# nexus1203/libBICOS

Measured on NVIDIA B200. Metric: Mpx/s disparity, higher is better.
Workload: dtype u8

## Files before the change

libbicos_b200/csrc/search_mma.cu:

```cuda

#include "kernels.cuh"

#include <atomic>
#include <limits.h>
#include <mutex>
#include <stdio.h>
#include <stdlib.h>
#include <string.h>

namespace bicos_b200 {
namespace {

constexpr int TM = 128;
constexpr int TN = 128;
constexpr int NTHREADS = 320;
constexpr int ATOM_BYTES = 128 * 128;
constexpr uint32_t TMEM_COLS = 2 * TN;
constexpr int COL_BITS = 13;
constexpr int COL_MAX = (1 << COL_BITS) - 1;
#ifndef BICOS_MMA_COLTERM_DEFAULT
#define BICOS_MMA_COLTERM_DEFAULT 1
#endif

__device__ __forceinline__ uint32_t smem_u32(const void* p) {
// ... 132 lines not shown
    asm volatile(
        "tcgen05.ld.sync.aligned.32x32b.x32.b32 {%0, %1, %2, %3, %4, %5, %6, %7, %8, %9, %10, %11, %12, %13, %14, %15, %16, %17, %18, %19, %20, %21, %22, %23, %24, %25, %26, %27, %28, %29, %30, %31}, [%32];"
        : "=r"(v[0]), "=r"(v[1]), "=r"(v[2]), "=r"(v[3]), "=r"(v[4]), "=r"(v[5]), "=r"(v[6]), "=r"(v[7]), "=r"(v[8]), "=r"(v[9]), "=r"(v[10]), "=r"(v[11]), "=r"(v[12]), "=r"(v[13]), "=r"(v[14]), "=r"(v[15]), "=r"(v[16]), "=r"(v[17]), "=r"(v[18]), "=r"(v[19]), "=r"(v[20]), "=r"(v[21]), "=r"(v[22]), "=r"(v[23]), "=r"(v[24]), "=r"(v[25]), "=r"(v[26]), "=r"(v[27]), "=r"(v[28]), "=r"(v[29]), "=r"(v[30]), "=r"(v[31])
        : "r"(taddr)
        : "memory"
    );
}

__device__ __forceinline__ void tc_load64_packed_issue(uint32_t taddr, int (&v)[32]) {
    asm volatile(
        "tcgen05.ld.sync.aligned.32x32b.x32.pack::16b.b32 {%0, %1, %2, %3, %4, %5, %6, %7, %8, %9, %10, %11, %12, %13, %14, %15, %16, %17, %18, %19, %20, %21, %22, %23, %24, %25, %26, %27, %28, %29, %30, %31}, [%32];"
        : "=r"(v[0]), "=r"(v[1]), "=r"(v[2]), "=r"(v[3]), "=r"(v[4]), "=r"(v[5]), "=r"(v[6]), "=r"(v[7]), "=r"(v[8]), "=r"(v[9]), "=r"(v[10]), "=r"(v[11]), "=r"(v[12]), "=r"(v[13]), "=r"(v[14]), "=r"(v[15]), "=r"(v[16]), "=r"(v[17]), "=r"(v[18]), "=r"(v[19]), "=r"(v[20]), "=r"(v[21]), "=r"(v[22]), "=r"(v[23]), "=r"(v[24]), "=r"(v[25]), "=r"(v[26]), "=r"(v[27]), "=r"(v[28]), "=r"(v[29]), "=r"(v[30]), "=r"(v[31])
        : "r"(taddr)
        : "memory"
    );
}

__device__ __forceinline__ void tc_load32_wait(int (&v)[32]) {
    asm volatile("tcgen05.wait::ld.sync.aligned;" : "+r"(v[0]), "+r"(v[1]), "+r"(v[2]), "+r"(v[3]), "+r"(v[4]), "+r"(v[5]), "+r"(v[6]), "+r"(v[7]), "+r"(v[8]), "+r"(v[9]), "+r"(v[10]), "+r"(v[11]), "+r"(v[12]), "+r"(v[13]), "+r"(v[14]), "+r"(v[15]), "+r"(v[16]), "+r"(v[17]), "+r"(v[18]), "+r"(v[19]), "+r"(v[20]), "+r"(v[21]), "+r"(v[22]), "+r"(v[23]), "+r"(v[24]), "+r"(v[25]), "+r"(v[26]), "+r"(v[27]), "+r"(v[28]), "+r"(v[29]), "+r"(v[30]), "+r"(v[31])::"memory");
}

__device__ __forceinline__ void tc_store32(uint32_t taddr, const uint32_t (&v)[32]) {
    asm volatile(
        "tcgen05.st.sync.aligned.32x32b.x32.b32 [%0], {%1, %2, %3, %4, %5, %6, %7, %8, %9, %10, %11, %12, %13, %14, %15, %16, %17, %18, %19, %20, %21, %22, %23, %24, %25, %26, %27, %28, %29, %30, %31, %32};"
        :
        : "r"(taddr), "r"(v[0]), "r"(v[1]), "r"(v[2]), "r"(v[3]), "r"(v[4]), "r"(v[5]), "r"(v[6]), "r"(v[7]), "r"(v[8]), "r"(v[9]), "r"(v[10]), "r"(v[11]), "r"(v[12]), "r"(v[13]), "r"(v[14]), "r"(v[15]), "r"(v[16]), "r"(v[17]), "r"(v[18]), "r"(v[19]), "r"(v[20]), "r"(v[21]), "r"(v[22]), "r"(v[23]), "r"(v[24]), "r"(v[25]), "r"(v[26]), "r"(v[27]), "r"(v[28]), "r"(v[29]), "r"(v[30]), "r"(v[31])
        : "memory"
    );
}

__device__ __forceinline__ void tc_store_wait() {
    asm volatile("tcgen05.wait::st.sync.aligned;" ::: "memory");
}

__device__ __forceinline__ void tc_mma_i8_ts(uint32_t tmem_d, uint32_t tmem_a, uint64_t bdesc, uint32_t idesc, uint32_t accumulate) {
    asm volatile(
        "{\n"
        ".reg .pred p;\n"
        "setp.ne.b32 p, %4, 0;\n"
        "tcgen05.mma.cta_group::1.kind::i8 [%0], [%1], %2, %3, p;\n"
        "}"
        :
        : "r"(tmem_d), "r"(tmem_a), "l"(bdesc), "r"(idesc), "r"(accumulate)
        : "memory"
    );
}

__device__ __forceinline__ uint64_t smem_desc(uint32_t saddr) {
    uint64_t d = (uint64_t)((saddr & 0x3FFFFu) >> 4);
    d |= (uint64_t)1 << 16;
    d |= (uint64_t)(1024 >> 4) << 32;
    d |= (uint64_t)1 << 46;
    d |= (uint64_t)2 << 61;
    return d;
}

constexpr uint32_t IDESC = (2u << 4) | (1u << 7) | (0u << 10) | ((uint32_t)(TN >> 3) << 17) | ((uint32_t)(TM >> 4) << 24);

__device__ __forceinline__ void st_shared_v4(uint32_t addr, uint32_t a, uint32_t b, uint32_t c, uint32_t d) {
    asm volatile("st.shared.v4.b32 [%0], {%1, %2, %3, %4};" ::"r"(addr), "r"(a), "r"(b), "r"(c), "r"(d) : "memory");
}

template<bool RIGHT, int S>
__device__ __forceinline__ uint32_t expand_word(uint32_t w) {
    if constexpr (RIGHT) {
        if constexpr (S == 0)
            return (w << 7) & 0x80808080u;
        else
            return w & (0x01010101u << S);
    } else {
        constexpr int P = S == 0 ? 0 : 7 - S;
        constexpr uint32_t MAG = 0x01010101u << P;
        constexpr uint32_t HIGH = 0x01010101u * ((0xFFu << (P + 1)) & 0xFFu);
        const uint32_t neg = ((w >> S) & 0x01010101u) * 0xFFu;
        return (neg & HIGH) | MAG;
    }
}

template<int K, bool RIGHT, bool CT = false>
__device__ __forceinline__ void expand_pixel(const uint4 (&d)[K / 4], uint32_t tile, int r) {
    const uint32_t row = tile + (uint32_t)r * 128u;
    const uint32_t sw = (uint32_t)(r & 7);
#pragma unroll
    for (int q = 0; q < K / 4; ++q) {
        const uint32_t w[4] = { d[q].x, d[q].y, d[q].z, d[q].w };
#pragma unroll
        for (int wi = 0; wi < 4; ++wi) {
            st_shared_v4(
                row + (uint32_t)q * ATOM_BYTES + ((((uint32_t)(2 * wi)) ^ sw) << 4),
                expand_word<RIGHT, 0>(w[wi]),
                expand_word<RIGHT, 1>(w[wi]),
                expand_word<RIGHT, 2>(w[wi]),
                expand_word<RIGHT, 3>(w[wi])
            );
            st_shared_v4(
                row + (uint32_t)q * ATOM_BYTES + ((((uint32_t)(2 * wi + 1)) ^ sw) << 4),
                expand_word<RIGHT, 4>(w[wi]),
                expand_word<RIGHT, 5>(w[wi]),
                expand_word<RIGHT, 6>(w[wi]),
                (RIGHT && CT && q == K / 4 - 1 && wi == 3) ? (expand_word<RIGHT, 7>(w[wi]) | ((uint32_t)r << 24)) : expand_word<RIGHT, 7>(w[wi])
            );
        }
    }
}

template<int K>
// ... 666 lines not shown
                    TileMin16 m;
                    tc_load64_packed_issue(acc, va);
                    tc_load64_packed_issue(acc + 64, vb);
                    tc_load32_wait(va);
                    tc_load32_wait(vb);
                    tc_fence_before();
                    mbar_arrive(bar_acc_drained + 8 * (2 * a + h));
                    fold64_packed<NODUPES, 0, CT>(va, m);
                    fold64_packed<NODUPES, 64, CT>(vb, m);
                    merge_tile<NODUPES>(m, tile0, m_first, m_last);
                } else {
                    TileMin32 m;
                    tc_load32_issue(acc, va);
                    tc_load32_wait(va);
                    tc_load32_issue(acc + 32, vb);
                    fold32<NODUPES, 0, CT>(va, m);
                    tc_load32_wait(vb);
                    tc_load32_issue(acc + 64, va);
                    fold32<NODUPES, 32, CT>(vb, m);
                    tc_load32_wait(va);
                    tc_load32_issue(acc + 96, vb);
                    fold32<NODUPES, 64, CT>(va, m);
                    tc_load32_wait(vb);
                    tc_fence_before();
                    mbar_arrive(bar_acc_drained + 8 * (2 * a + h));
                    fold32<NODUPES, 96, CT>(vb, m);
                    merge_tile<NODUPES>(m, tile0, m_first, m_last);
                }
                if (n + 1 < nitems && t == (NA == 2 ? min(2, ntiles - 1) : ntiles - 1))
                    pa_next = stage_left(dl, n + 1);
            }
            const int i = it.mt * 2 * TM + h * TM + lane128;
            if (i < cols) {
                const size_t at = (size_t)it.row * cols + i;
                (it.dir ? p.rev_first : p.fwd_first)[at] = ((uint32_t)(pa + (m_first >> COL_BITS)) << 16) | ((uint32_t)m_first & COL_MAX);
                if constexpr (NODUPES)
                    (it.dir ? p.rev_last : p.fwd_last)[at] =
                        ((uint32_t)(pa + (m_last >> COL_BITS)) << 16) | ((65535u - COL_MAX) + ((uint32_t)m_last & COL_MAX));
            }
            it = nx;
        }
    }

teardown:
    tc_fence_before();
    __syncthreads();
    if (warp == 1) {
        tc_fence_after();
        asm volatile("tcgen05.dealloc.cta_group::1.sync.aligned.b32 %0, %1;" ::"r"(*(volatile uint32_t*)&tmem_base_slot), "r"(512u) : "memory");
    }
}

constexpr int V3_THREADS = 512;
template<int K>
constexpr int V3_REGS_LAUNCH = K == 4 ? 104 : 112;
constexpr int V3_REGS_EPILOGUE = 168;
template<int K>
constexpr int V3_REGS_PRODUCER = K == 4 ? 40 : 56;
template<int K>
constexpr int V3_REGS_ISSUER = K == 4 ? 40 : 56;
template<int K>
constexpr bool V3_REGS_FIT = 256 * V3_REGS_EPILOGUE + 128 * V3_REGS_PRODUCER<K> + 128 * V3_REGS_ISSUER<K> <= V3_THREADS * V3_REGS_LAUNCH<K>;
static_assert(V3_REGS_FIT<4> && V3_REGS_FIT<8>, "register budget");
template<int K>
constexpr int V3_ASLOTS = K == 4 ? 4 : 2;
constexpr int V3_PACKED = 4;
constexpr uint32_t V3_A_COL0 = 3 * TN;
template<int K>
constexpr int V3_PACKED_BYTES = TN * K * 4;
template<int K>
constexpr int V3_OFFSET = K == 4 ? 0 : 16384;
constexpr int V3_STATE_STRIDE = 132;
constexpr int V3_STATE_BYTES = 64 * V3_STATE_STRIDE * 4;
constexpr int V3_FIN_BYTES = 2 * TN * 4;
template<int K>
constexpr int V3_SMEM_BYTES = 4 * (K / 4) * ATOM_BYTES + V3_PACKED * V3_PACKED_BYTES<K> + 2 * V3_STATE_BYTES + 2 * V3_FIN_BYTES + 1024;
static_assert(V3_SMEM_BYTES<8> <= 227 * 1024, "shared memory");
constexpr uint32_t IDESC3 = (2u << 4) | (0u << 7) | (1u << 10) | ((uint32_t)(TN >> 3) << 17) | ((uint32_t)(TM >> 4) << 24);

__device__ __forceinline__ void tc_store8(uint32_t taddr, const uint32_t (&v)[8]) {
    asm volatile("tcgen05.st.sync.aligned.32x32b.x8.b32 [%0], {%1, %2, %3, %4, %5, %6, %7, %8};" ::"r"(taddr), "r"(v[0]), "r"(v[1]), "r"(v[2]),
                 "r"(v[3]), "r"(v[4]), "r"(v[5]), "r"(v[6]), "r"(v[7])
                 : "memory");
}

__device__ __forceinline__ void st_shared_v2(uint32_t addr, uint32_t a, uint32_t b) {
    asm volatile("st.shared.v2.b32 [%0], {%1, %2};" ::"r"(addr), "r"(a), "r"(b) : "memory");
}
__device__ __forceinline__ void st_shared_u32(uint32_t addr, uint32_t a) {
    asm volatile("st.shared.b32 [%0], %1;" ::"r"(addr), "r"(a) : "memory");
}
__device__ __forceinline__ uint32_t ld_shared_u32(uint32_t addr) {
    uint32_t v;
    asm volatile("ld.shared.b32 %0, [%1];" : "=r"(v) : "r"(addr) : "memory");
    return v;
}
__device__ __forceinline__ uint32_t pinned(uint32_t v) {
    uint32_t r;
    asm volatile("mov.u32 %0, %1;" : "=r"(r) : "r"(v));
    return r;
}

template<int K>
__device__ __forceinline__ void expand_moving_to_tmem(const uint4 (&d)[K / 4], uint32_t taddr) {
#pragma unroll
    for (int q = 0; q < K / 4; ++q) {
    const uint32_t w[4] = { d[q].x, d[q].y, d[q].z, d[q].w };
#pragma unroll
    for (int wi = 0; wi < 4; ++wi) {
        uint32_t v[8];
        v[0] = expand_word<true, 0>(w[wi]);
        v[1] = expand_word<true, 1>(w[wi]);
        v[2] = expand_word<true, 2>(w[wi]);
        v[3] = expand_word<true, 3>(w[wi]);
        v[4] = expand_word<true, 4>(w[wi]);
        v[5] = expand_word<true, 5>(w[wi]);
        v[6] = expand_word<true, 6>(w[wi]);
        v[7] = expand_word<true, 7>(w[wi]);
        if (q == K / 4 - 1 && wi == 3) {
            v[6] |= 128u << 24;
            v[7] |= 1u << 24;
        }
        tc_store8(taddr + 32u * q + 8u * wi, v);
    }
    }
    tc_store_wait();
}

template<int K>
__device__ __forceinline__ void expand_block_pixel(const uint4 (&d)[K / 4], uint32_t tile, int r) {
    const uint32_t row = tile + (uint32_t)r * 128u;
    const uint32_t sw = (uint32_t)(r & 7);
    int pc = 0;
#pragma unroll
    for (int q = 0; q < K / 4; ++q)
        pc += __popc(d[q].x) + __popc(d[q].y) + __popc(d[q].z) + __popc(d[q].w);
    const uint32_t pc_byte = (uint32_t)(pc - (K == 4 ? 0 : 128)) & 0xFFu;
#pragma unroll
    for (int q = 0; q < K / 4; ++q) {
        const uint32_t w[4] = { d[q].x, d[q].y, d[q].z, d[q].w };
        const uint32_t atom = row + (uint32_t)q * ATOM_BYTES;
#pragma unroll
        for (int wi = 0; wi < 4; ++wi) {
            st_shared_v4(atom + ((((uint32_t)(2 * wi)) ^ sw) << 4), expand_word<false, 0>(w[wi]), expand_word<false, 1>(w[wi]),
                         expand_word<false, 2>(w[wi]), expand_word<false, 3>(w[wi]));
            uint32_t s6 = expand_word<false, 6>(w[wi]), s7 = expand_word<false, 7>(w[wi]);
            if (q == K / 4 - 1 && wi == 3) {
                s6 = (s6 & 0x00FFFFFFu) | (pc_byte << 24);
                s7 = (s7 & 0x00FFFFFFu) | ((uint32_t)r << 24);
            }
            st_shared_v4(atom + ((((uint32_t)(2 * wi + 1)) ^ sw) << 4), expand_word<false, 4>(w[wi]), expand_word<false, 5>(w[wi]), s6, s7);
        }
    }
}

template<int L>
__device__ __forceinline__ uint32_t key_of_hi(uint32_t w, uint32_t mask) {
    uint32_t k;
    asm("lop3.b32 %0, %1, %2, %3, 0xEA;" : "=r"(k) : "r"(w), "r"(mask), "n"(L));
    return k;
}
template<int L4>
struct ReduceLanes {
    static __device__ __forceinline__ void run(uint32_t src, uint32_t mask, uint32_t shl16, uint32_t& mlo, uint32_t& mhi) {
        const uint4 w = ld_shared_v4(src + 16u * L4);
        mhi = min(mhi, min(key_of_hi<4 * L4>(w.x, mask), key_of_hi<4 * L4 + 1>(w.y, mask)));
        mlo = min(mlo, min(w.x * shl16 + (uint32_t)(4 * L4), w.y * shl16 + (uint32_t)(4 * L4 + 1)));
        mhi = min(mhi, min(key_of_hi<4 * L4 + 2>(w.z, mask), key_of_hi<4 * L4 + 3>(w.w, mask)));
        mlo = min(mlo, min(w.z * shl16 + (uint32_t)(4 * L4 + 2), w.w * shl16 + (uint32_t)(4 * L4 + 3)));
        ReduceLanes<L4 + 1>::run(src, mask, shl16, mlo, mhi);
    }
};
template<>
struct ReduceLanes<16> {
    static __device__ __forceinline__ void run(uint32_t, uint32_t, uint32_t, uint32_t&, uint32_t&) {}
};

#define V3_ROLE_CONTEXT \
    uint32_t fresh; \
    asm volatile("mov.u32 %0, 0;" : "=r"(fresh)); \
    const uint32_t tmem = *(volatile uint32_t*)&tmem_base_slot + fresh; \
    const int cols = p.cols; \
    const int ntiles = p.ntiles;  \
    const int npairs = p.mtiles;  \
    const long long item0 = p.items * (blockIdx.x + fresh) / gridDim.x; \
    const int nitems = (int)(p.items * (blockIdx.x + fresh + 1) / gridDim.x - item0); \
    const uint32_t s_blk = ((smem_u32(smem_raw) + fresh) + 1023u) & ~1023u;  \
    const uint32_t s_packed = s_blk + 4 * BLK_BYTES; \
    const uint32_t s_state = s_packed + NP * PACKED_BYTES;  \
    const uint32_t s_fin = s_state + 2 * V3_STATE_BYTES;  \
    const uint32_t bar_packed_full = smem_u32(&bars[0]) + fresh; \
    const uint32_t bar_packed_free = bar_packed_full + 8 * NP; \
    const uint32_t bar_a_full = bar_packed_free + 8 * NP; \
    const uint32_t bar_a_free = bar_a_full + 8 * NS; \
    const uint32_t bar_blk_full = bar_a_free + 8 * NS;  \
    const uint32_t bar_blk_free = bar_blk_full + 32; \
    const uint32_t bar_acc_full = bar_blk_free + 32; \
    const uint32_t bar_acc_drained = bar_acc_full + 48; \
    const uint32_t bar_epi = bar_acc_drained + 48;  \
    int row = (int)(item0 / npairs), bp = (int)(item0 - (long long)row * npairs); \
    (void)tmem, (void)cols, (void)ntiles, (void)s_blk, (void)s_packed, (void)s_state, (void)s_fin, (void)bar_packed_full, (void)bar_packed_free, \
        (void)bar_a_full, (void)bar_a_free, (void)bar_blk_full, (void)bar_blk_free, (void)bar_acc_full, (void)bar_acc_drained, (void)bar_epi, \
        (void)row, (void)bp;

template<int K>
__global__ void __maxnreg__(V3_REGS_LAUNCH<K>) search_mma3_kernel(const MmaArgs p) {
    constexpr int KA = K / 4;
    constexpr int NS = V3_ASLOTS<K>;
    constexpr int NP = V3_PACKED;
    constexpr int PACKED_BYTES = V3_PACKED_BYTES<K>;
    constexpr int BLK_BYTES = KA * ATOM_BYTES;
    constexpr uint32_t A_COLS = 32u * KA;
    constexpr int OFF = V3_OFFSET<K>;
    extern __shared__ uint8_t smem_raw[];
    __shared__ uint64_t bars[2 * NP + 2 * NS + 8 + 12 + 2];
    __shared__ uint32_t tmem_base_slot;
    __shared__ Watch s_watch;

    const int tid = threadIdx.x;
    const int warp = tid >> 5;

    if (tid == 0) {
        const uint32_t bar0 = smem_u32(&bars[0]);
        s_watch.flag = p.timeout_flag;
        s_watch.timeout_ns = p.timeout_ns;
        s_watch.abort = 0;
        for (int s = 0; s < NP; ++s) {
            mbar_init(bar0 + 8 * s, 1);
            mbar_init(bar0 + 8 * (NP + s), TM);
        }
        for (int s = 0; s < NS; ++s) {
            mbar_init(bar0 + 8 * (2 * NP + s), TM);
            mbar_init(bar0 + 8 * (2 * NP + NS + s), 2);
        }
        for (int b = 0; b < 4; ++b) {
            mbar_init(bar0 + 8 * (2 * NP + 2 * NS + b), TN);
            mbar_init(bar0 + 8 * (2 * NP + 2 * NS + 4 + b), 1);
        }
        for (int a = 0; a < 6; ++a) {
            mbar_init(bar0 + 8 * (2 * NP + 2 * NS + 8 + a), 1);
            mbar_init(bar0 + 8 * (2 * NP + 2 * NS + 14 + a), TM);
        }
        mbar_init(bar0 + 8 * (2 * NP + 2 * NS + 20), TM);
        mbar_init(bar0 + 8 * (2 * NP + 2 * NS + 21), TM);
        asm volatile("fence.mbarrier_init.release.cluster;" ::: "memory");
    }
    if (warp == 1) {
        asm volatile("tcgen05.alloc.cta_group::1.sync.aligned.shared::cta.b32 [%0], %1;" ::"r"(smem_u32(&tmem_base_slot)), "r"(512u)
                     : "memory");
        asm volatile("tcgen05.relinquish_alloc_permit.cta_group::1.sync.aligned;" ::: "memory");
    }
    tc_fence_before();
    __syncthreads();
    tc_fence_after();

    if (warp >= 12) {
        regs_shrink<V3_REGS_ISSUER<K>>();
        V3_ROLE_CONTEXT
    if (warp == 15) {
    } else if (warp == 12 || warp == 13) {
        {
            const int h = warp - 12;
            const uint32_t u_tmem = uniform(tmem);
            const uint64_t desc_b0 = smem_desc(uniform(s_blk)) + (uint32_t)h * (uint32_t)(BLK_BYTES >> 4);
            constexpr uint32_t BUFFER_STEP = (2 * BLK_BYTES) >> 4;
            uint32_t s = 0, a_phase = 0;
            uint32_t a = (uint32_t)h, d6 = (uint32_t)h + 3u, d_phase = 1u;
            int q = h;
            for (int n = 0; n < nitems; ++n) {
                const uint32_t b = (uint32_t)n & 1u;
                if (!mbar_wait(bar_blk_full + 8 * (2 * b + h), ((uint32_t)n >> 1) & 1u, &s_watch))
                    goto teardown;
                const uint64_t desc_b = desc_b0 + b * BUFFER_STEP;
                for (int t = 0; t < ntiles; ++t, q += 2) {
                    if (!mbar_wait(bar_a_full + 8 * s, a_phase, &s_watch))
                        goto teardown;
                    if (q >= 3)
                        if (!mbar_wait(bar_acc_drained + 8 * (2 * a + (1 - h)), d_phase, &s_watch))
                            goto teardown;
                    tc_fence_after();
                    if (elect_one()) {
#pragma unroll
                        for (int qa = 0; qa < KA; ++qa)
#pragma unroll
                            for (int kk = 0; kk < 4; ++kk)
                                tc_mma_i8_ts(u_tmem + a * TN, u_tmem + V3_A_COL0 + s * A_COLS + (uint32_t)(qa * 32 + kk * 8),
                                             desc_b + (uint32_t)((qa * ATOM_BYTES + kk * 32) >> 4), IDESC3, (qa | kk) != 0);
                        tc_commit(bar_acc_full + 8 * (2 * a + h));
                        tc_commit(bar_a_free + 8 * s);
                    }
                    __syncwarp();
                    if (++s == NS) {
                        s = 0;
                        a_phase ^= 1u;
                    }
                    a = a == 0 ? 2u : a - 1u;
                    d6 += 2u;
                    if (d6 >= 6u) {
                        d6 -= 6u;
                        d_phase ^= 1u;
                    }
                }
                if (elect_one())
                    tc_commit(bar_blk_free + 8 * (2 * b + h));
                __syncwarp();
            }
        }
    } else if (warp == 14) {
        if (tid == 14 * 32) {
            uint32_t slot = 0, free_phase = 1u;
            bool wrapped = false;
            const uint32_t tail_bytes = (uint32_t)(cols - (ntiles - 1) * TN) * (uint32_t)(K * 4);
            auto put = [&](const uint32_t* src, uint32_t bytes) -> bool {
                if (wrapped)
                    if (!mbar_wait(bar_packed_free + 8 * slot, free_phase, &s_watch))
                        return false;
                mbar_expect_tx(bar_packed_full + 8 * slot, bytes);
                bulk_copy_g2s(s_packed + slot * (uint32_t)PACKED_BYTES, src, bytes, bar_packed_full + 8 * slot);
                if (++slot == (uint32_t)NP) {
                    slot = 0;
                    free_phase ^= 1u;
                    wrapped = true;
                }
                return true;
            };
            for (int n = 0; n < nitems; ++n) {
                const uint32_t* const lrow = p.left + (size_t)row * p.pitch_words;
                const uint32_t* const rrow = p.right + (size_t)row * p.pitch_words;
                for (int e = 0; e < 2; ++e) {
                    const int base = min((2 * bp + e) * TN, cols - 1);
                    if (!put(rrow + (size_t)base * K, (uint32_t)min(TN, cols - base) * (uint32_t)(K * 4)))
                        goto teardown;
                }
                for (int t = 0; t < ntiles - 1; ++t)
                    if (!put(lrow + (size_t)t * (TN * K), (uint32_t)PACKED_BYTES))
                        goto teardown;
                if (!put(lrow + (size_t)(ntiles - 1) * (TN * K), tail_bytes))
                    goto teardown;
                if (++bp == npairs) {
                    bp = 0;
                    ++row;
                }
            }
        }
    }
    } else if (warp >= 8) {
        regs_shrink<V3_REGS_PRODUCER<K>>();
        V3_ROLE_CONTEXT
        const int r = (int)pinned((uint32_t)(tid - 2 * TM));
        const uint32_t lane_base = tmem + ((uint32_t)((warp & 3) * 32) << 16);
        uint32_t ps = 0, full_phase = 0, as = 0, a_free_phase = 1u;
        bool a_wrapped = false;
        const uint32_t my_px = s_packed + (uint32_t)r * (uint32_t)(K * 4);
        const uint32_t my_tail_px = s_packed + (uint32_t)min(r, cols - (ntiles - 1) * TN - 1) * (uint32_t)(K * 4);
        for (int n = 0; n < nitems; ++n) {
            for (int e = 0; e < 2; ++e) {
                const int valid = min(TN, cols - min((2 * bp + e) * TN, cols - 1));
                if (!mbar_wait(bar_packed_full + 8 * ps, full_phase, &s_watch))
                    goto teardown;
                uint4 d[KA];
                {
                    const uint32_t src = s_packed + ps * (uint32_t)PACKED_BYTES + (uint32_t)min(r, valid - 1) * (uint32_t)(K * 4);
#pragma unroll
                    for (int q = 0; q < KA; ++q)
                        d[q] = ld_shared_v4(src + 16u * q);
                }
                const uint32_t b = 2u * ((uint32_t)n & 1u) + (uint32_t)e;
                if (n >= 2)
                    if (!mbar_wait(bar_blk_free + 8 * b, (((uint32_t)n >> 1) - 1u) & 1u, &s_watch))
                        goto teardown;
                expand_block_pixel<K>(d, s_blk + b * BLK_BYTES, r);
                mbar_arrive(bar_packed_free + 8 * ps);
                fence_async_smem();
                mbar_arrive(bar_blk_full + 8 * b);
                if (++ps == (uint32_t)NP) {
                    ps = 0;
                    full_phase ^= 1u;
                }
            }
            for (int t = 0; t < ntiles; ++t) {
                if (!mbar_wait(bar_packed_full + 8 * ps, full_phase, &s_watch))
                    goto teardown;
                uint4 d[KA];
                {
                    const uint32_t src = (t == ntiles - 1 ? my_tail_px : my_px) + ps * (uint32_t)PACKED_BYTES;
#pragma unroll
                    for (int q = 0; q < KA; ++q)
                        d[q] = ld_shared_v4(src + 16u * q);
                }
                if (a_wrapped)
                    if (!mbar_wait(bar_a_free + 8 * as, a_free_phase, &s_watch))
                        goto teardown;
                tc_fence_after();
                expand_moving_to_tmem<K>(d, lane_base + V3_A_COL0 + as * A_COLS);
                mbar_arrive(bar_packed_free + 8 * ps);
                tc_fence_before();
                mbar_arrive(bar_a_full + 8 * as);
                if (++ps == (uint32_t)NP) {
                    ps = 0;
                    full_phase ^= 1u;
                }
                if (++as == (uint32_t)NS) {
                    as = 0;
                    a_free_phase ^= 1u;
                    a_wrapped = true;
                }
            }
            if (++bp == npairs) {
                bp = 0;
                ++row;
            }
        }
    } else {
        regs_grow<V3_REGS_EPILOGUE>();
        V3_ROLE_CONTEXT
        const int h = (int)pinned((uint32_t)(warp >> 2));
        const int lane128 = (int)pinned((uint32_t)(tid & (TM - 1)));
        const uint32_t lane_base = tmem + ((uint32_t)((warp & 3) * 32) << 16);
        const uint32_t my_state = s_state + (uint32_t)(h * V3_STATE_BYTES);
        const uint32_t my_fin = s_fin + (uint32_t)(h * V3_FIN_BYTES);
        const uint32_t my_epi = bar_epi + 8u * (uint32_t)h;
        uint32_t R[64];
#pragma unroll
        for (int c = 0; c < 64; ++c)
            R[c] = 0x7FFF7FFFu;
        uint32_t epi_phase = 0;
        uint32_t a = (uint32_t)h, acc_phase = 0;
        int lo[32], hi[32];
        int left = nitems * ntiles;
        if (left > 0) {
            if (!mbar_wait(bar_acc_full + 8 * (2 * a + h), acc_phase, &s_watch))
                goto teardown;
            tc_fence_after();
            tc_load64_packed_issue(lane_base + a * TN, lo);
            --left;
        }
        for (int n = 0; n < nitems; ++n) {
            const size_t row_at = (size_t)row * cols;
            const int col0 = (2 * bp + h) * TN;
            const int fwd_cols = col0 < cols ? cols : 0;
            for (int t = 0; t < ntiles; ++t) {
                const uint32_t tile2 = (uint32_t)(t + OFF) * 0x00010001u;
                uint32_t f[8];
                tc_load32_wait(lo);
                tc_load64_packed_issue(lane_base + a * TN + 64u, hi);
#pragma unroll
                for (int c = 0; c < 8; ++c)
                    f[c] = __vimin3_s16x2((uint32_t)lo[c], (uint32_t)lo[8 + c], (uint32_t)lo[16 + c]);
#pragma unroll
                for (int c = 0; c < 4; ++c)
                    f[c] = __vimin3_s16x2(f[c], (uint32_t)lo[24 + 2 * c], (uint32_t)lo[25 + 2 * c]);
#pragma unroll
                for (int c = 0; c < 32; ++c)
                    R[c] = __viaddmin_s16x2((uint32_t)lo[c], tile2, R[c]);
                tc_load32_wait(hi);
                tc_fence_before();
                mbar_arrive(bar_acc_drained + 8 * (2 * a + h));
                a = a == 0 ? 2u : a - 1u;
                if (a == (uint32_t)h)
                    acc_phase ^= 1u;
                if (left > 0) {
                    if (!mbar_wait(bar_acc_full + 8 * (2 * a + h), acc_phase, &s_watch))
                        goto teardown;
                    tc_fence_after();
                    tc_load64_packed_issue(lane_base + a * TN, lo);
                    --left;
                }
#pragma unroll
                for (int c = 0; c < 8; ++c)
                    f[c] = __vimin3_s16x2(f[c], (uint32_t)hi[c], (uint32_t)hi[8 + c]);
#pragma unroll
                for (int c = 0; c < 8; ++c)
                    f[c] = __vimin3_s16x2(f[c], (uint32_t)hi[16 + c], (uint32_t)hi[24 + c]);
                const uint32_t m2 = __vimin3_s16x2(__vimin3_s16x2(f[0], f[1], f[2]), __vimin3_s16x2(f[3], f[4], f[5]), __vmins2(f[6], f[7]));
                const uint32_t m = OFF ? (uint32_t)(min((int)(short)(m2 & 0xFFFFu), (int)(short)(m2 >> 16)) + OFF) : min(m2 & 0xFFFFu, m2 >> 16);
                const int i = t * TM + lane128;
                if (i < fwd_cols)
                    atomicMin(p.fwd_first + row_at + i, m * 512u + (uint32_t)col0 - (m & 127u) * 511u);
#pragma unroll
                for (int c = 0; c < 32; ++c)
                    R[32 + c] = __viaddmin_s16x2((uint32_t)hi[c], tile2, R[32 + c]);
            }
            {
                const uint32_t dst = my_state + (uint32_t)(lane128 * 4);
#pragma unroll
                for (int c = 0; c < 64; ++c) {
                    st_shared_u32(dst + (uint32_t)(c * V3_STATE_STRIDE * 4), R[c]);
                    R[c] = 0x7FFF7FFFu;
                }
                mbar_arrive(my_epi);
                if (!mbar_wait(my_epi, epi_phase, &s_watch))
                    goto teardown;
                epi_phase ^= 1u;
                const int cp = lane128 & 63, lh = lane128 >> 6;
                const uint32_t src = my_state + (uint32_t)((cp * V3_STATE_STRIDE + lh * 64) * 4);
                uint32_t mlo = 0xFFFFFFFFu, mhi = 0xFFFFFFFFu;
                ReduceLanes<0>::run(src, pinned(0xFFFF0000u), pinned(65536u), mlo, mhi);
                const uint32_t lane0 = (uint32_t)lh * 64u;
                st_shared_v2(my_fin + (uint32_t)((lh * TN + 2 * cp) * 4), mlo + lane0, mhi + lane0);
                mbar_arrive(my_epi);
                if (!mbar_wait(my_epi, epi_phase, &s_watch))
                    goto teardown;
                epi_phase ^= 1u;
                {
                    const int col = col0 + lane128;
                    const uint32_t k = min(ld_shared_u32(my_fin + (uint32_t)(lane128 * 4)), ld_shared_u32(my_fin + (uint32_t)((TN + lane128) * 4)));
                    const uint32_t vv = (k >> 16) - (uint32_t)lane128;
                    if (col < cols)
                        p.rev_first[row_at + col] = ((vv >> 7) << 16) | ((vv & 127u) * TM + (k & 0xFFFFu));
                }
            }
            if (++bp == npairs) {
                bp = 0;
                ++row;
            }
        }
    }

teardown:
    tc_fence_before();
    __syncthreads();
    if (warp == 1) {
        tc_fence_after();
        asm volatile("tcgen05.dealloc.cta_group::1.sync.aligned.b32 %0, %1;" ::"r"(*(volatile uint32_t*)&tmem_base_slot), "r"(512u) : "memory");
    }
}

int sm_count_of_current_device() {
    static thread_local int cached_dev = -1, cached_sms = 148;
    int dev = 0;
    if (cudaGetDevice(&dev) == cudaSuccess && dev != cached_dev) {
        if (cudaDeviceGetAttribute(&cached_sms, cudaDevAttrMultiProcessorCount, dev) != cudaSuccess)
            cached_sms = 148;
        cached_dev = dev;
// ... 18 lines not shown
            break;
        }
    if (e && e->kernel == kernel && dev < 64 && ((e->devices >> dev) & 1ull))
        return cudaSuccess;
    if ((err = cudaFuncSetAttribute(kernel, cudaFuncAttributeMaxDynamicSharedMemorySize, smem)) != cudaSuccess)
        return err;
    if ((err = cudaFuncSetAttribute(kernel, cudaFuncAttributePreferredSharedMemoryCarveout, cudaSharedmemCarveoutMaxShared)) != cudaSuccess)
        return err;
    if (e && dev < 64) {
        e->kernel = kernel;
        e->devices |= 1ull << dev;
    }
    return cudaSuccess;
}

template<int K>
constexpr int v2_smem_bytes() {
    return V2_STAGES<K> * (K / 4) * ATOM_BYTES + V2_PACKED * TN * K * 4 + 1024;
}

template<int K, bool NODUPES, bool CT>
cudaError_t launch_k2(MmaArgs p, int dirs, cudaStream_t stream) {
    constexpr int smem = v2_smem_bytes<K>();
    auto kernel = search_mma2_kernel<K, NODUPES, CT>;
    cudaError_t err = configure_once(kernel, smem);
    if (err != cudaSuccess)
        return err;
    const int sms = sm_count_of_current_device();
    p.mtiles = (p.cols + 2 * TM - 1) / (2 * TM);
    p.items = (long long)dirs * p.rows * p.mtiles;
    if (p.items > 0x7FFFFFFFLL)
        return cudaErrorInvalidConfiguration;
    const unsigned grid = (unsigned)(p.items < sms ? p.items : sms);
    kernel<<<grid, V2_THREADS, smem, stream>>>(p);
    return cudaGetLastError();
}

template<int K, bool NODUPES, bool CT>
cudaError_t launch_k(MmaArgs p, int dirs, cudaStream_t stream) {
    const int smem = search_mma_smem_bytes(K);
    auto kernel = search_mma_kernel<K, NODUPES, CT>;
    cudaError_t err = configure_once(kernel, smem);
    if (err != cudaSuccess)
        return err;
    const int resident = sm_count_of_current_device() * (K <= 8 ? 2 : 1);
    p.items = (long long)dirs * p.rows * p.mtiles;
    if (p.items > 0x7FFFFFFFLL)
        return cudaErrorInvalidConfiguration;
    const unsigned grid = (unsigned)(p.items < resident ? p.items : resident);
    kernel<<<grid, NTHREADS, smem, stream>>>(p);
    return cudaGetLastError();
}

template<int K>
cudaError_t launch_k3(MmaArgs p, cudaStream_t stream) {
    auto kernel = search_mma3_kernel<K>;
    constexpr int smem = V3_SMEM_BYTES<K>;
    cudaError_t err = configure_once(kernel, smem);
    if (err != cudaSuccess)
        return err;
    p.mtiles = (p.cols + 2 * TN - 1) / (2 * TN);
    p.items = (long long)p.rows * p.mtiles;
    if (p.items > 0x7FFFFFFFLL)
        return cudaErrorInvalidConfiguration;
    if ((err = cudaMemsetAsync(p.fwd_first, 0xFF, (size_t)p.rows * p.cols * sizeof(uint32_t), stream)) != cudaSuccess)
        return err;
    const int sms = sm_count_of_current_device();
    const unsigned grid = (unsigned)(p.items < sms ? p.items : sms);
    kernel<<<grid, V3_THREADS, smem, stream>>>(p);
    return cudaGetLastError();
}

}

int search_mma_smem_bytes(int K) {
    const int stages = K == 4 ? STAGES<4> : K == 8 ? STAGES<8> : K == 12 ? STAGES<12> : STAGES<16>;
    const int lefts = K == 4 ? LEFT_BUFFERS<4> : 1;
    const int packed = K == 4 ? PACKED_STAGES<4> : K == 8 ? PACKED_STAGES<8> : PACKED_STAGES<16>;
    return (lefts + stages) * (K / 4) * ATOM_BYTES + packed * TN * K * 4 + 1024;
}

namespace {
std::atomic<int> g_variant { -1 };
std::atomic<int> g_colterm { -1 };
std::atomic<long long> g_timeout_ms { -1 };
std::atomic<unsigned int*> g_timeout_flag { nullptr };
std::mutex g_timeout_mutex;

unsigned int* mma_timeout_flag() {
    unsigned int* f = g_timeout_flag.load(std::memory_order_acquire);
    if (f)
        return f;
    std::lock_guard<std::mutex> lk(g_timeout_mutex);
    f = g_timeout_flag.load(std::memory_order_acquire);
    if (!f) {
        void* p = nullptr;
        if (cudaHostAlloc(&p, 64, cudaHostAllocPortable | cudaHostAllocMapped) != cudaSuccess) {
            cudaGetLastError();
            return nullptr;
        }
        memset(p, 0, 64);
        f = static_cast<unsigned int*>(p);
        g_timeout_flag.store(f, std::memory_order_release);
    }
    return f;
}

unsigned long long mma_timeout_ns() {
    long long ms = g_timeout_ms.load(std::memory_order_relaxed);
    if (ms < 0) {
        const char* v = getenv("BICOS_B200_MMA_TIMEOUT_MS");
        ms = v ? atoll(v) : 0;
        if (ms <= 0)
            ms = 10000;
        g_timeout_ms.store(ms, std::memory_order_relaxed);
    }
    return (unsigned long long)ms * 1000000ull;
}
}

unsigned int search_mma_take_timeout() {
    unsigned int* f = g_timeout_flag.load(std::memory_order_acquire);
    if (!f)
        return 0;
    const unsigned int v = *(volatile unsigned int*)f;
    if (v)
        *(volatile unsigned int*)f = 0;
    return v;
}

int search_mma_variant() {
    int g = g_variant.load(std::memory_order_relaxed);
    if (g < 0) {
        const char* v = getenv("BICOS_B200_MMA_VARIANT");
        g = v && v[0] == '3' ? 3 : v && v[0] == '2' ? 2 : v && v[0] == '1' ? 1 : 0;
        g_variant.store(g, std::memory_order_relaxed);
    }
    return g;
}

void set_search_mma_variant(int v) {
    g_variant.store(v >= 1 && v <= 3 ? v : 0, std::memory_order_relaxed);
}

bool search_mma_colterm() {
    int g = g_colterm.load(std::memory_order_relaxed);
    if (g < 0) {
        const char* v = getenv("BICOS_B200_MMA_COLTERM");
        g = v ? (v[0] == '1') : BICOS_MMA_COLTERM_DEFAULT;
        g_colterm.store(g, std::memory_order_relaxed);
    }
    return g == 1;
}

void set_search_mma_colterm(bool on) {
    g_colterm.store(on ? 1 : 0, std::memory_order_relaxed);
}

bool search_mma_onepass_applies(int K, int cols, int flags, int free_top_bits) {
    const int variant = search_mma_variant();
    return (K == 4 || K == 8) && cols >= 1 && cols <= COL_MAX + 1 && flags == FLAG_CONSISTENCY && free_top_bits >= 2
        && (variant == 3 || variant == 0) && search_mma_colterm();
}

bool search_mma_supports(int K, int cols) {
    return (K == 4 || K == 8 || K == 12 || K == 16) && cols >= 1 && cols <= COL_MAX + 1;
}

cudaError_t launch_search_mma(
    const uint32_t* desc0,
    const uint32_t* desc1,
    int K,
    int rows,
    int cols,
    size_t desc_pitch_words,
    int flags,
    uint32_t* fwd_first,
    uint32_t* fwd_last,
    uint32_t* rev_first,
    uint32_t* rev_last,
    cudaStream_t stream,
    int free_top_bits
) {
    const bool top_bit_free = free_top_bits >= 1;
    if (rows <= 0 || !search_mma_supports(K, cols))
        return cudaErrorInvalidValue;
    if ((((uintptr_t)desc0 | (uintptr_t)desc1) & 15) != 0 || (desc_pitch_words & 3) != 0)
        return cudaErrorMisalignedAddress;
    MmaArgs p;
    p.left = desc0;
    p.right = desc1;
    p.rows = rows;
    p.cols = cols;
    p.pitch_words = desc_pitch_words;
    p.mtiles = (cols + TM - 1) / TM;
    p.ntiles = (cols + TN - 1) / TN;
    p.fwd_first = fwd_first;
    p.fwd_last = fwd_last;
    p.rev_first = rev_first;
    p.rev_last = rev_last;
    p.timeout_flag = mma_timeout_flag();
    p.timeout_ns = mma_timeout_ns();
    const int dirs = (flags & FLAG_CONSISTENCY) ? 2 : 1;
    const bool nodupes = (flags & FLAG_NODUPES) != 0;
    const long long pair_items = (long long)dirs * rows * ((cols + 2 * TM - 1) / (2 * TM));
    const int variant = search_mma_variant();
    if (search_mma_onepass_applies(K, cols, flags, free_top_bits)) {
        note_search_kernel("mma3<K=%d,nodupes=0,ct=2,onepass=1>", K);
        return K == 4 ? launch_k3<4>(p, stream) : launch_k3<8>(p, stream);
    }
    const bool v2 = (K == 4 || K == 8) && (variant == 2 || (variant == 0 && pair_items >= 2 * sm_count_of_current_device()));
    const bool ct = top_bit_free && (K == 4 || K == 8) && search_mma_colterm();
    note_search_kernel("mma%d<K=%d,nodupes=%d,ct=%d,dirs=%d>", v2 ? 2 : 1, K, (int)nodupes, (int)ct, dirs);
#define BICOS_MMA_DISPATCH(LAUNCH, KK)                                                                      \
    (ct ? (nodupes ? LAUNCH<KK, true, true>(p, dirs, stream) : LAUNCH<KK, false, true>(p, dirs, stream))      \
        : (nodupes ? LAUNCH<KK, true, false>(p, dirs, stream) : LAUNCH<KK, false, false>(p, dirs, stream)))
    if (v2 && K == 4)
        return BICOS_MMA_DISPATCH(launch_k2, 4);
    if (v2 && K == 8)
        return BICOS_MMA_DISPATCH(launch_k2, 8);
    switch (K) {
        case 4:
            return BICOS_MMA_DISPATCH(launch_k, 4);
        case 8:
            return BICOS_MMA_DISPATCH(launch_k, 8);
        case 12:
            return nodupes ? launch_k<12, true, false>(p, dirs, stream) : launch_k<12, false, false>(p, dirs, stream);
        case 16:
            return nodupes ? launch_k<16, true, false>(p, dirs, stream) : launch_k<16, false, false>(p, dirs, stream);
    }
#undef BICOS_MMA_DISPATCH
    return cudaErrorInvalidValue;
}

}
```

Before: 2013.

## Fold per-tile bias into an extra MMA for the K=4 one-pass kernel

```diff
diff --git a/libbicos_b200/csrc/search_mma.cu b/libbicos_b200/csrc/search_mma.cu
--- a/libbicos_b200/csrc/search_mma.cu
+++ b/libbicos_b200/csrc/search_mma.cu
@@ -208,6 +208,12 @@
     d |= (uint64_t)(1024 >> 4) << 32;
     d |= (uint64_t)1 << 46;
     d |= (uint64_t)2 << 61;
+    return d;
+}
+
+__device__ __forceinline__ uint64_t smem_desc_rows_repeated(uint32_t saddr) {
+    uint64_t d = (uint64_t)((saddr & 0x3FFFFu) >> 4);
+    d |= (uint64_t)1 << 46;
     return d;
 }
 
@@ -980,16 +986,18 @@
 }
 
 constexpr int V3_THREADS = 512;
-template<int K>
-constexpr int V3_REGS_LAUNCH = K == 4 ? 104 : 112;
-constexpr int V3_REGS_EPILOGUE = 168;
-template<int K>
+template<int K, bool BIAS>
+constexpr int V3_REGS_LAUNCH = BIAS ? 128 : K == 4 ? 104 : 112;
+template<bool BIAS>
+constexpr int V3_REGS_EPILOGUE = BIAS ? 216 : 168;
+template<int K, bool BIAS>
 constexpr int V3_REGS_PRODUCER = K == 4 ? 40 : 56;
-template<int K>
+template<int K, bool BIAS>
 constexpr int V3_REGS_ISSUER = K == 4 ? 40 : 56;
-template<int K>
-constexpr bool V3_REGS_FIT = 256 * V3_REGS_EPILOGUE + 128 * V3_REGS_PRODUCER<K> + 128 * V3_REGS_ISSUER<K> <= V3_THREADS * V3_REGS_LAUNCH<K>;
-static_assert(V3_REGS_FIT<4> && V3_REGS_FIT<8>, "register budget");
+template<int K, bool BIAS>
+constexpr bool V3_REGS_FIT = 256 * V3_REGS_EPILOGUE<BIAS> + 128 * V3_REGS_PRODUCER<K, BIAS> + 128 * V3_REGS_ISSUER<K, BIAS> <= V3_THREADS * V3_REGS_LAUNCH<K, BIAS>;
+static_assert(V3_REGS_FIT<4, false> && V3_REGS_FIT<4, true> && V3_REGS_FIT<8, false>, "register budget");
+static_assert(V3_THREADS * V3_REGS_LAUNCH<4, true> <= 65536, "register file");
 template<int K>
 constexpr int V3_ASLOTS = K == 4 ? 4 : 2;
 constexpr int V3_PACKED = 4;
@@ -998,12 +1006,17 @@
 constexpr int V3_PACKED_BYTES = TN * K * 4;
 template<int K>
 constexpr int V3_OFFSET = K == 4 ? 0 : 16384;
+template<bool BIAS>
+constexpr int V3_CHUNK_BYTES = BIAS ? ATOM_BYTES : 0;
 constexpr int V3_STATE_STRIDE = 132;
 constexpr int V3_STATE_BYTES = 64 * V3_STATE_STRIDE * 4;
 constexpr int V3_FIN_BYTES = 2 * TN * 4;
-template<int K>
-constexpr int V3_SMEM_BYTES = 4 * (K / 4) * ATOM_BYTES + V3_PACKED * V3_PACKED_BYTES<K> + 2 * V3_STATE_BYTES + 2 * V3_FIN_BYTES + 1024;
-static_assert(V3_SMEM_BYTES<8> <= 227 * 1024, "shared memory");
+constexpr int V3_MAX_TILES = (COL_MAX + 1) / TN;
+template<bool BIAS>
+constexpr int V3_TABLE_BYTES = BIAS ? V3_MAX_TILES * 128 : 0;
+template<int K, bool BIAS>
+constexpr int V3_SMEM_BYTES = 4 * (K / 4) * ATOM_BYTES + 4 * V3_CHUNK_BYTES<BIAS> + V3_PACKED * V3_PACKED_BYTES<K> + 2 * V3_STATE_BYTES + 2 * V3_FIN_BYTES + V3_TABLE_BYTES<BIAS> + 1024;
+static_assert(V3_SMEM_BYTES<8, false> <= 227 * 1024 && V3_SMEM_BYTES<4, true> <= 227 * 1024, "shared memory");
 constexpr uint32_t IDESC3 = (2u << 4) | (0u << 7) | (1u << 10) | ((uint32_t)(TN >> 3) << 17) | ((uint32_t)(TM >> 4) << 24);
 
 __device__ __forceinline__ void tc_store8(uint32_t taddr, const uint32_t (&v)[8]) {
@@ -1029,7 +1042,7 @@
     return r;
 }
 
-template<int K>
+template<int K, bool BIAS>
 __device__ __forceinline__ void expand_moving_to_tmem(const uint4 (&d)[K / 4], uint32_t taddr) {
 #pragma unroll
     for (int q = 0; q < K / 4; ++q) {
@@ -1045,7 +1058,7 @@
         v[5] = expand_word<true, 5>(w[wi]);
         v[6] = expand_word<true, 6>(w[wi]);
         v[7] = expand_word<true, 7>(w[wi]);
-        if (q == K / 4 - 1 && wi == 3) {
+        if (!BIAS && q == K / 4 - 1 && wi == 3) {
             v[6] |= 128u << 24;
             v[7] |= 1u << 24;
         }
@@ -1055,8 +1068,8 @@
     tc_store_wait();
 }
 
-template<int K>
-__device__ __forceinline__ void expand_block_pixel(const uint4 (&d)[K / 4], uint32_t tile, int r) {
+template<int K, bool BIAS>
+__device__ __forceinline__ void expand_block_pixel(const uint4 (&d)[K / 4], uint32_t tile, uint32_t chunk, int r) {
     const uint32_t row = tile + (uint32_t)r * 128u;
     const uint32_t sw = (uint32_t)(r & 7);
     int pc = 0;
@@ -1064,6 +1077,11 @@
     for (int q = 0; q < K / 4; ++q)
         pc += __popc(d[q].x) + __popc(d[q].y) + __popc(d[q].z) + __popc(d[q].w);
     const uint32_t pc_byte = (uint32_t)(pc - (K == 4 ? 0 : 128)) & 0xFFu;
+    if constexpr (BIAS) {
+        const uint32_t crow = chunk + (uint32_t)r * 128u;
+        st_shared_v4(crow + (sw << 4), pc_byte | ((uint32_t)r << 8) | (1u << 16), 0u, 0u, 0u);
+        st_shared_v4(crow + ((1u ^ sw) << 4), 0u, 0u, 0u, 0u);
+    }
 #pragma unroll
     for (int q = 0; q < K / 4; ++q) {
         const uint32_t w[4] = { d[q].x, d[q].y, d[q].z, d[q].w };
@@ -1073,7 +1091,7 @@
             st_shared_v4(atom + ((((uint32_t)(2 * wi)) ^ sw) << 4), expand_word<false, 0>(w[wi]), expand_word<false, 1>(w[wi]),
                          expand_word<false, 2>(w[wi]), expand_word<false, 3>(w[wi]));
             uint32_t s6 = expand_word<false, 6>(w[wi]), s7 = expand_word<false, 7>(w[wi]);
-            if (q == K / 4 - 1 && wi == 3) {
+            if (!BIAS && q == K / 4 - 1 && wi == 3) {
                 s6 = (s6 & 0x00FFFFFFu) | (pc_byte << 24);
                 s7 = (s7 & 0x00FFFFFFu) | ((uint32_t)r << 24);
             }
@@ -1103,6 +1121,24 @@
 struct ReduceLanes<16> {
     static __device__ __forceinline__ void run(uint32_t, uint32_t, uint32_t, uint32_t&, uint32_t&) {}
 };
+
+__device__ __forceinline__ void fold_forward_lo(uint32_t (&f)[8], const int (&lo)[32]) {
+#pragma unroll
+    for (int c = 0; c < 8; ++c)
+        f[c] = __vimin3_s16x2((uint32_t)lo[c], (uint32_t)lo[8 + c], (uint32_t)lo[16 + c]);
+#pragma unroll
+    for (int c = 0; c < 4; ++c)
+        f[c] = __vimin3_s16x2(f[c], (uint32_t)lo[24 + 2 * c], (uint32_t)lo[25 + 2 * c]);
+}
+__device__ __forceinline__ uint32_t fold_forward_hi(uint32_t (&f)[8], const int (&hi)[32]) {
+#pragma unroll
+    for (int c = 0; c < 8; ++c)
+        f[c] = __vimin3_s16x2(f[c], (uint32_t)hi[c], (uint32_t)hi[8 + c]);
+#pragma unroll
+    for (int c = 0; c < 8; ++c)
+        f[c] = __vimin3_s16x2(f[c], (uint32_t)hi[16 + c], (uint32_t)hi[24 + c]);
+    return __vimin3_s16x2(__vimin3_s16x2(f[0], f[1], f[2]), __vimin3_s16x2(f[3], f[4], f[5]), __vmins2(f[6], f[7]));
+}
 
 #define V3_ROLE_CONTEXT \
     uint32_t fresh; \
@@ -1114,7 +1150,8 @@
     const long long item0 = p.items * (blockIdx.x + fresh) / gridDim.x; \
     const int nitems = (int)(p.items * (blockIdx.x + fresh + 1) / gridDim.x - item0); \
     const uint32_t s_blk = ((smem_u32(smem_raw) + fresh) + 1023u) & ~1023u;  \
-    const uint32_t s_packed = s_blk + 4 * BLK_BYTES; \
+    const uint32_t s_chunk = s_blk + 4 * BLK_BYTES;  \
+    const uint32_t s_packed = s_chunk + 4 * CHUNK_BYTES; \
     const uint32_t s_state = s_packed + NP * PACKED_BYTES;  \
     const uint32_t s_fin = s_state + 2 * V3_STATE_BYTES;  \
     const uint32_t bar_packed_full = smem_u32(&bars[0]) + fresh; \
@@ -1127,18 +1164,22 @@
     const uint32_t bar_acc_drained = bar_acc_full + 48; \
     const uint32_t bar_epi = bar_acc_drained + 48;  \
     int row = (int)(item0 / npairs), bp = (int)(item0 - (long long)row * npairs); \
-    (void)tmem, (void)cols, (void)ntiles, (void)s_blk, (void)s_packed, (void)s_state, (void)s_fin, (void)bar_packed_full, (void)bar_packed_free, \
+    (void)tmem, (void)cols, (void)ntiles, (void)s_blk, (void)s_chunk, (void)s_packed, (void)s_state, (void)s_fin, (void)bar_packed_full, (void)bar_packed_free, \
         (void)bar_a_full, (void)bar_a_free, (void)bar_blk_full, (void)bar_blk_free, (void)bar_acc_full, (void)bar_acc_drained, (void)bar_epi, \
         (void)row, (void)bp;
 
-template<int K>
-__global__ void __maxnreg__(V3_REGS_LAUNCH<K>) search_mma3_kernel(const MmaArgs p) {
+template<int K, bool BIAS>
+__global__ void __maxnreg__((V3_REGS_LAUNCH<K, BIAS>)) search_mma3_kernel(const MmaArgs p) {
+    static_assert(!BIAS || K == 4, "the bias chunk is laid out for 128-bit descriptors");
     constexpr int KA = K / 4;
     constexpr int NS = V3_ASLOTS<K>;
     constexpr int NP = V3_PACKED;
     constexpr int PACKED_BYTES = V3_PACKED_BYTES<K>;
     constexpr int BLK_BYTES = KA * ATOM_BYTES;
+    constexpr int CHUNK_BYTES = V3_CHUNK_BYTES<BIAS>;
     constexpr uint32_t A_COLS = 32u * KA;
+    constexpr int TABLE_BYTES = V3_TABLE_BYTES<BIAS>;
+    constexpr uint32_t TABLE_OFFSET = 4 * BLK_BYTES + 4 * CHUNK_BYTES + NP * PACKED_BYTES + 2 * V3_STATE_BYTES + 2 * V3_FIN_BYTES;
     constexpr int OFF = V3_OFFSET<K>;
     extern __shared__ uint8_t smem_raw[];
     __shared__ uint64_t bars[2 * NP + 2 * NS + 8 + 12 + 2];
@@ -1178,20 +1219,26 @@
                      : "memory");
         asm volatile("tcgen05.relinquish_alloc_permit.cta_group::1.sync.aligned;" ::: "memory");
     }
+    if constexpr (TABLE_BYTES > 0) {
+        static_assert(TABLE_BYTES / 16 == V3_THREADS, "one 16-byte row per thread");
+        const uint32_t s_table0 = ((smem_u32(smem_raw) + 1023u) & ~1023u) + TABLE_OFFSET;
+        st_shared_v4(s_table0 + 16u * (uint32_t)tid, 128u | (1u << 8) | ((uint32_t)(tid >> 3) << 16), 0u, 0u, 0u);
+        fence_async_smem();
+    }
     tc_fence_before();
     __syncthreads();
     tc_fence_after();
 
     if (warp >= 12) {
-        regs_shrink<V3_REGS_ISSUER<K>>();
+        regs_shrink<V3_REGS_ISSUER<K, BIAS>>();
         V3_ROLE_CONTEXT
     if (warp == 15) {
     } else if (warp == 12 || warp == 13) {
         {
             const int h = warp - 12;
             const uint32_t u_tmem = uniform(tmem);
-            const uint64_t desc_b0 = smem_desc(uniform(s_blk)) + (uint32_t)h * (uint32_t)(BLK_BYTES >> 4);
-            constexpr uint32_t BUFFER_STEP = (2 * BLK_BYTES) >> 4;
+            static_assert(!BIAS || CHUNK_BYTES == BLK_BYTES, "chunk tiles are indexed as the block tiles");
+            constexpr uint32_t CHUNK_FROM_BLOCK = (4 * BLK_BYTES) >> 4;
             uint32_t s = 0, a_phase = 0;
             uint32_t a = (uint32_t)h, d6 = (uint32_t)h + 3u, d_phase = 1u;
             int q = h;
@@ -1199,7 +1246,9 @@
                 const uint32_t b = (uint32_t)n & 1u;
                 if (!mbar_wait(bar_blk_full + 8 * (2 * b + h), ((uint32_t)n >> 1) & 1u, &s_watch))
                     goto teardown;
-                const uint64_t desc_b = desc_b0 + b * BUFFER_STEP;
+                const uint64_t desc_b = smem_desc(uniform(s_blk + (2u * b + (uint32_t)h) * (uint32_t)BLK_BYTES));
+                const uint64_t desc_table = smem_desc_rows_repeated(uniform(s_blk + TABLE_OFFSET));
+                (void)desc_table;
                 for (int t = 0; t < ntiles; ++t, q += 2) {
                     if (!mbar_wait(bar_a_full + 8 * s, a_phase, &s_watch))
                         goto teardown;
@@ -1214,6 +1263,8 @@
                             for (int kk = 0; kk < 4; ++kk)
                                 tc_mma_i8_ts(u_tmem + a * TN, u_tmem + V3_A_COL0 + s * A_COLS + (uint32_t)(qa * 32 + kk * 8),
                                              desc_b + (uint32_t)((qa * ATOM_BYTES + kk * 32) >> 4), IDESC3, (qa | kk) != 0);
+                        if constexpr (BIAS)
+                            tc_mma_i8(u_tmem + a * TN, desc_table + (uint32_t)(t * (128 >> 4)), desc_b + CHUNK_FROM_BLOCK, IDESC3, 1u);
                         tc_commit(bar_acc_full + 8 * (2 * a + h));
                         tc_commit(bar_a_free + 8 * s);
                     }
@@ -1273,7 +1324,7 @@
         }
     }
     } else if (warp >= 8) {
-        regs_shrink<V3_REGS_PRODUCER<K>>();
+        regs_shrink<V3_REGS_PRODUCER<K, BIAS>>();
         V3_ROLE_CONTEXT
         const int r = (int)pinned((uint32_t)(tid - 2 * TM));
         const uint32_t lane_base = tmem + ((uint32_t)((warp & 3) * 32) << 16);
@@ -1297,7 +1348,7 @@
                 if (n >= 2)
                     if (!mbar_wait(bar_blk_free + 8 * b, (((uint32_t)n >> 1) - 1u) & 1u, &s_watch))
                         goto teardown;
-                expand_block_pixel<K>(d, s_blk + b * BLK_BYTES, r);
+                expand_block_pixel<K, BIAS>(d, s_blk + b * BLK_BYTES, s_chunk + b * CHUNK_BYTES, r);
                 mbar_arrive(bar_packed_free + 8 * ps);
                 fence_async_smem();
                 mbar_arrive(bar_blk_full + 8 * b);
@@ -1320,7 +1371,7 @@
                     if (!mbar_wait(bar_a_free + 8 * as, a_free_phase, &s_watch))
                         goto teardown;
                 tc_fence_after();
-                expand_moving_to_tmem<K>(d, lane_base + V3_A_COL0 + as * A_COLS);
+                expand_moving_to_tmem<K, BIAS>(d, lane_base + V3_A_COL0 + as * A_COLS);
                 mbar_arrive(bar_packed_free + 8 * ps);
                 tc_fence_before();
                 mbar_arrive(bar_a_full + 8 * as);
@@ -1340,7 +1391,7 @@
             }
         }
     } else {
-        regs_grow<V3_REGS_EPILOGUE>();
+        regs_grow<V3_REGS_EPILOGUE<BIAS>>();
         V3_ROLE_CONTEXT
         const int h = (int)pinned((uint32_t)(warp >> 2));
         const int lane128 = (int)pinned((uint32_t)(tid & (TM - 1)));
@@ -1355,7 +1406,23 @@
         uint32_t epi_phase = 0;
         uint32_t a = (uint32_t)h, acc_phase = 0;
         int lo[32], hi[32];
+        int lo2[32], hi2[32];
         int left = nitems * ntiles;
+        auto next_tile = [&](int (&dst)[32]) -> bool {
+            tc_fence_before();
+            mbar_arrive(bar_acc_drained + 8 * (2 * a + h));
+            a = a == 0 ? 2u : a - 1u;
+            if (a == (uint32_t)h)
+                acc_phase ^= 1u;
+            if (left > 0) {
+                if (!mbar_wait(bar_acc_full + 8 * (2 * a + h), acc_phase, &s_watch))
+                    return false;
+                tc_fence_after();
+                tc_load64_packed_issue(lane_base + a * TN, dst);
+                --left;
+            }
+            return true;
+        };
         if (left > 0) {
             if (!mbar_wait(bar_acc_full + 8 * (2 * a + h), acc_phase, &s_watch))
                 goto teardown;
@@ -1367,47 +1434,72 @@
             const size_t row_at = (size_t)row * cols;
             const int col0 = (2 * bp + h) * TN;
             const int fwd_cols = col0 < cols ? cols : 0;
-            for (int t = 0; t < ntiles; ++t) {
-                const uint32_t tile2 = (uint32_t)(t + OFF) * 0x00010001u;
-                uint32_t f[8];
-                tc_load32_wait(lo);
-                tc_load64_packed_issue(lane_base + a * TN + 64u, hi);
-#pragma unroll
-                for (int c = 0; c < 8; ++c)
-                    f[c] = __vimin3_s16x2((uint32_t)lo[c], (uint32_t)lo[8 + c], (uint32_t)lo[16 + c]);
-#pragma unroll
-                for (int c = 0; c < 4; ++c)
-                    f[c] = __vimin3_s16x2(f[c], (uint32_t)lo[24 + 2 * c], (uint32_t)lo[25 + 2 * c]);
-#pragma unroll
-                for (int c = 0; c < 32; ++c)
-                    R[c] = __viaddmin_s16x2((uint32_t)lo[c], tile2, R[c]);
-                tc_load32_wait(hi);
-                tc_fence_before();
-                mbar_arrive(bar_acc_drained + 8 * (2 * a + h));
-                a = a == 0 ? 2u : a - 1u;
-                if (a == (uint32_t)h)
-                    acc_phase ^= 1u;
-                if (left > 0) {
-                    if (!mbar_wait(bar_acc_full + 8 * (2 * a + h), acc_phase, &s_watch))
-                        goto teardown;
-                    tc_fence_after();
-                    tc_load64_packed_issue(lane_base + a * TN, lo);
-                    --left;
-                }
-#pragma unroll
-                for (int c = 0; c < 8; ++c)
-                    f[c] = __vimin3_s16x2(f[c], (uint32_t)hi[c], (uint32_t)hi[8 + c]);
-#pragma unroll
-                for (int c = 0; c < 8; ++c)
-                    f[c] = __vimin3_s16x2(f[c], (uint32_t)hi[16 + c], (uint32_t)hi[24 + c]);
-                const uint32_t m2 = __vimin3_s16x2(__vimin3_s16x2(f[0], f[1], f[2]), __vimin3_s16x2(f[3], f[4], f[5]), __vmins2(f[6], f[7]));
-                const uint32_t m = OFF ? (uint32_t)(min((int)(short)(m2 & 0xFFFFu), (int)(short)(m2 >> 16)) + OFF) : min(m2 & 0xFFFFu, m2 >> 16);
+            auto forward = [&](uint32_t m2, int t) {
+                const uint32_t m = OFF ? (uint32_t)(min((int)(short)(m2 & 0xFFFFu), (int)(short)(m2 >> 16)) + OFF)
+                                       : min(m2 & 0xFFFFu, m2 >> 16) - (BIAS ? (uint32_t)t : 0u);
                 const int i = t * TM + lane128;
                 if (i < fwd_cols)
                     atomicMin(p.fwd_first + row_at + i, m * 512u + (uint32_t)col0 - (m & 127u) * 511u);
-#pragma unroll
-                for (int c = 0; c < 32; ++c)
-                    R[32 + c] = __viaddmin_s16x2((uint32_t)hi[c], tile2, R[32 + c]);
+            };
+            if constexpr (BIAS) {
+                int t = 0;
+                for (; t + 1 < ntiles; t += 2) {
+                    uint32_t f[8];
+                    tc_load32_wait(lo);
+                    tc_load64_packed_issue(lane_base + a * TN + 64u, hi);
+                    fold_forward_lo(f, lo);
+                    tc_load32_wait(hi);
+                    if (!next_tile(lo2))
+                        goto teardown;
+                    forward(fold_forward_hi(f, hi), t);
+                    tc_load32_wait(lo2);
+                    tc_load64_packed_issue(lane_base + a * TN + 64u, hi2);
+                    fold_forward_lo(f, lo2);
+#pragma unroll
+                    for (int c = 0; c < 32; ++c)
+                        R[c] = __vimin3_s16x2(R[c], (uint32_t)lo[c], (uint32_t)lo2[c]);
+                    tc_load32_wait(hi2);
+                    if (!next_tile(lo))
+                        goto teardown;
+                    forward(fold_forward_hi(f, hi2), t + 1);
+#pragma unroll
+                    for (int c = 0; c < 32; ++c)
+                        R[32 + c] = __vimin3_s16x2(R[32 + c], (uint32_t)hi[c], (uint32_t)hi2[c]);
+                }
+                if (t < ntiles) {
+                    uint32_t f[8];
+                    tc_load32_wait(lo);
+                    tc_load64_packed_issue(lane_base + a * TN + 64u, hi);
+                    fold_forward_lo(f, lo);
+#pragma unroll
+                    for (int c = 0; c < 32; ++c)
+                        R[c] = __vmins2(R[c], (uint32_t)lo[c]);
+                    tc_load32_wait(hi);
+                    if (!next_tile(lo))
+                        goto teardown;
+                    forward(fold_forward_hi(f, hi), t);
+#pragma unroll
+                    for (int c = 0; c < 32; ++c)
+                        R[32 + c] = __vmins2(R[32 + c], (uint32_t)hi[c]);
+                }
+            } else {
+                for (int t = 0; t < ntiles; ++t) {
+                    const uint32_t tile2 = (uint32_t)(t + OFF) * 0x00010001u;
+                    uint32_t f[8];
+                    tc_load32_wait(lo);
+                    tc_load64_packed_issue(lane_base + a * TN + 64u, hi);
+                    fold_forward_lo(f, lo);
+#pragma unroll
+                    for (int c = 0; c < 32; ++c)
+                        R[c] = __viaddmin_s16x2((uint32_t)lo[c], tile2, R[c]);
+                    tc_load32_wait(hi);
+                    if (!next_tile(lo))
+                        goto teardown;
+                    forward(fold_forward_hi(f, hi), t);
+#pragma unroll
+                    for (int c = 0; c < 32; ++c)
+                        R[32 + c] = __viaddmin_s16x2((uint32_t)hi[c], tile2, R[32 + c]);
+                }
             }
             {
                 const uint32_t dst = my_state + (uint32_t)(lane128 * 4);
@@ -1532,10 +1624,10 @@
     return cudaGetLastError();
 }
 
-template<int K>
+template<int K, bool BIAS>
 cudaError_t launch_k3(MmaArgs p, cudaStream_t stream) {
-    auto kernel = search_mma3_kernel<K>;
-    constexpr int smem = V3_SMEM_BYTES<K>;
+    auto kernel = search_mma3_kernel<K, BIAS>;
+    constexpr int smem = V3_SMEM_BYTES<K, BIAS>;
     cudaError_t err = configure_once(kernel, smem);
     if (err != cudaSuccess)
         return err;
@@ -1613,14 +1705,14 @@
     int g = g_variant.load(std::memory_order_relaxed);
     if (g < 0) {
         const char* v = getenv("BICOS_B200_MMA_VARIANT");
-        g = v && v[0] == '3' ? 3 : v && v[0] == '2' ? 2 : v && v[0] == '1' ? 1 : 0;
+        g = v && v[0] >= '1' && v[0] <= '4' ? v[0] - '0' : 0;
         g_variant.store(g, std::memory_order_relaxed);
     }
     return g;
 }
 
 void set_search_mma_variant(int v) {
-    g_variant.store(v >= 1 && v <= 3 ? v : 0, std::memory_order_relaxed);
+    g_variant.store(v >= 1 && v <= 4 ? v : 0, std::memory_order_relaxed);
 }
 
 bool search_mma_colterm() {
@@ -1640,7 +1732,7 @@
 bool search_mma_onepass_applies(int K, int cols, int flags, int free_top_bits) {
     const int variant = search_mma_variant();
     return (K == 4 || K == 8) && cols >= 1 && cols <= COL_MAX + 1 && flags == FLAG_CONSISTENCY && free_top_bits >= 2
-        && (variant == 3 || variant == 0) && search_mma_colterm();
+        && (variant == 0 || variant >= 3) && search_mma_colterm();
 }
 
 bool search_mma_supports(int K, int cols) {
@@ -1686,8 +1778,16 @@
     const long long pair_items = (long long)dirs * rows * ((cols + 2 * TM - 1) / (2 * TM));
     const int variant = search_mma_variant();
     if (search_mma_onepass_applies(K, cols, flags, free_top_bits)) {
-        note_search_kernel("mma3<K=%d,nodupes=0,ct=2,onepass=1>", K);
-        return K == 4 ? launch_k3<4>(p, stream) : launch_k3<8>(p, stream);
+        if (K == 8) {
+            note_search_kernel("mma3<K=8,nodupes=0,ct=2,onepass=1>");
+            return launch_k3<8, false>(p, stream);
+        }
+        if (variant == 4) {
+            note_search_kernel("mma3<K=4,nodupes=0,ct=2,onepass=1,bias=0>");
+            return launch_k3<4, false>(p, stream);
+        }
+        note_search_kernel("mma3<K=4,nodupes=0,ct=2,onepass=1>");
+        return launch_k3<4, true>(p, stream);
     }
     const bool v2 = (K == 4 || K == 8) && (variant == 2 || (variant == 0 && pair_items >= 2 * sm_count_of_current_device()));
     const bool ct = top_bit_free && (K == 4 || K == 8) && search_mma_colterm();
```

Measured after the change: 2035 (median of 6 runs). 1.01x the previous value.
